# slothfulxtx/Texture-GS

Hardware: AMD Instinct MI355X
Metric: fwd+bwd views/sec @800x800, 300k Gaussians + 1024^2 texture; HBM GB/s vs roofline (higher is better)
Workload: dtype f32; 1 GPU; c3: N=300000 Gaussians, cubemap 6x1024x1024x3 f32, 800x800, fwd+bwd, sh_degree 3; parallelism=views sharded dp1, view_pipeline=3 HIP streams, order=accumulate, forwards begun one view per stream ahead, grad_allreduce=none (1 GPU)

## Files before the change

### texture-gs_amd/build.py

```python
import os
import subprocess
import sys

HERE = os.path.dirname(os.path.abspath(__file__))
ROOT = os.path.dirname(HERE)
CSRC = os.path.join(HERE, "csrc")
OBJ = os.path.join(HERE, "build")
LIB = os.path.join(HERE, os.environ.get("TEXGS_LIB_NAME", "libtexgs.so"))
OBJ = os.path.join(HERE, os.environ.get("TEXGS_OBJ_DIR", "build"))
HIPCC = os.environ.get("HIPCC", "/opt/rocm/bin/hipcc")

COMMON = ["--offload-arch=gfx950", "-O3", "-std=c++17", "-fPIC", "-I" + os.path.join(ROOT, "include"),
          "-I" + CSRC, "-Wall"]
UNITS = {
    "preprocess.hip": ["-ffp-contract=off"],
    "binning.hip": [],
    "render.hip": ["-munsafe-fp-atomics", "-ffp-contract=fast", "-fno-slp-vectorize"],
    "loss.hip": [],
    "selftest.hip": [],
    "uvnet.hip": [],
    "uvmap.hip": ["-munsafe-fp-atomics"],
    "points.hip": ["-ffp-contract=off"],
    "cubetex.hip": ["-munsafe-fp-atomics"],
    "density.hip": ["-ffp-contract=off"],
    "metrics.hip": ["-ffp-contract=off"],
    "optim.hip": ["-ffp-contract=off"],
    "mlp.hip": [],
    "present.hip": ["-ffp-contract=off"],
    "abi.hip": [],
}
HEADERS = [os.path.join(CSRC, "common.h"), os.path.join(CSRC, "wave_ops.h"), os.path.join(CSRC, "render_bwd_body.h"),
           os.path.join(ROOT, "include", "texgs.h"), os.path.join(ROOT, "include", "texgs_optim.h"),
           os.path.join(ROOT, "include", "texgs_multiview.h"), os.path.join(ROOT, "include", "texgs_mlp.h"),
           os.path.join(ROOT, "include", "texgs_present.h")]


def build_id():
    import hashlib
    h = hashlib.sha256()
    files = sorted(os.path.join(CSRC, f) for f in os.listdir(CSRC) if f.endswith((".hip", ".h"))) \
        + [os.path.join(ROOT, "include", f) for f in ("texgs.h", "texgs_optim.h", "texgs_multiview.h", "texgs_mlp.h", "texgs_present.h")]
    for f in files:
        h.update(os.path.basename(f).encode())
        h.update(open(f, "rb").read())
    h.update(repr((COMMON[:4], sorted(UNITS.items()), os.environ.get("TEXGS_EXTRA_FLAGS", ""))).encode())
    return h.hexdigest()[:16]


def _newer(src_list, target):
    if not os.path.exists(target):
        return True
    t = os.path.getmtime(target)
    return any(os.path.getmtime(s) > t for s in src_list)


def build(force=False, verbose=False):
    os.makedirs(OBJ, exist_ok=True)
    objs = []
    bid = build_id()
    idfile = os.path.join(OBJ, "build_id.txt")
    stale_id = not os.path.exists(idfile) or open(idfile).read().strip() != bid
    for src, flags in UNITS.items():
        sp = os.path.join(CSRC, src)
        op = os.path.join(OBJ, src.replace(".hip", ".o"))
        objs.append(op)
        if src == "abi.hip":
            flags = flags + ['-DTEXGS_BUILD_ID="%s"' % bid]
        if force or _newer([sp] + HEADERS + [os.path.abspath(__file__)], op) or (src == "abi.hip" and stale_id):
            cmd = [HIPCC] + COMMON + flags + os.environ.get("TEXGS_EXTRA_FLAGS", "").split() + ["-c", sp, "-o", op]
            if verbose:
                print(" ".join(cmd), flush=True)
            subprocess.check_call(cmd)
    if force or _newer(objs, LIB):
        cmd = [HIPCC, "--offload-arch=gfx950", "-shared", "-fPIC", "-o", LIB] + objs
        if verbose:
            print(" ".join(cmd), flush=True)
        subprocess.check_call(cmd)
    with open(idfile, "w") as f:
        f.write(bid + "\n")
    return LIB


if __name__ == "__main__":
    print(build(force="--force" in sys.argv, verbose="--verbose" in sys.argv or True))
```

### texture-gs_amd/csrc/abi.hip

```cpp
#include "common.h"
#include <stdio.h>
#include <stdlib.h>

#include <mutex>
#include <vector>

namespace {

thread_local char g_err[512] = "";

struct EvRec { int kid; hipEvent_t a, b; };
std::mutex g_prof_mu;
bool g_prof_on = false;
uint32_t g_prof_mask = 0xFFFFFFFFu;
std::vector<EvRec> g_prof_log;
std::vector<hipEvent_t> g_prof_free;

hipEvent_t prof_event() {
    if (!g_prof_free.empty()) { hipEvent_t e = g_prof_free.back(); g_prof_free.pop_back(); return e; }
    hipEvent_t e = nullptr;
    return hipEventCreate(&e) == hipSuccess ? e : nullptr;
}

struct ProfScope {
    int kid; hipStream_t s; hipEvent_t a; bool on;
    ProfScope(int k, hipStream_t st) : kid(k), s(st), a(nullptr), on(false) {
        std::lock_guard<std::mutex> l(g_prof_mu);
        if (g_prof_on && ((g_prof_mask >> k) & 1u)) { a = prof_event(); on = a != nullptr; if (on) (void)hipEventRecord(a, s); }
    }
    ~ProfScope() {
        if (!on) return;
        std::lock_guard<std::mutex> l(g_prof_mu);
        hipEvent_t b = prof_event();
        if (!b) { g_prof_free.push_back(a); return; }
        (void)hipEventRecord(b, s);
        g_prof_log.push_back({kid, a, b});
    }
};

int fail(const char* where, hipError_t e) {
    snprintf(g_err, sizeof(g_err), "%s: %s", where, hipGetErrorString(e));
    return (int)e ? (int)e : -1;
}

int fail_msg(const char* msg) {
    snprintf(g_err, sizeof(g_err), "%s", msg);
    return -1;
}

int launched(const char* where, hipError_t st, hipStream_t s, bool debug) {
    if (st == hipSuccess && debug) st = hipStreamSynchronize(s);
    return st == hipSuccess ? 0 : fail(where, st);
}

int validate_frame(const TexGSFrame* f) {
    if (!f) return fail_msg("frame is NULL");
    if (f->image_height <= 0 || f->image_width <= 0) return fail_msg("image size must be positive");
    if (f->image_width > 65535 * TEXGS_TILE || f->image_height > 65535 * TEXGS_TILE) return fail_msg("image too large");
    {
        const long long tx = (f->image_width + TEXGS_TILE - 1) / TEXGS_TILE, ty = (f->image_height + TEXGS_TILE - 1) / TEXGS_TILE;
        if (tx * ty > (1ll << 24)) return fail_msg("image too large: more than 2^24 tiles");
    }
    if (f->sh_degree < 0 || f->sh_degree > 3) return fail_msg("sh_degree must be in [0,3]");
    if (f->num_gaussians < 0) return fail_msg("num_gaussians < 0");
    if (f->tex_res <= 0) return fail_msg("tex_res must be positive");
    if (f->tex_res > 7168) return fail_msg("tex_res > 7168: the blend kernels address texels with 32-bit byte offsets (6 R^2 x 12 B < 2^32)");
    if (!f->bg || !f->viewmatrix || !f->projmatrix || !f->campos) return fail_msg("frame device pointers must be non-NULL");
    return 0;
}

}

extern "C" {

int texgs_abi_version(void) { return TEXGS_ABI_VERSION; }

#ifndef TEXGS_BUILD_ID
#define TEXGS_BUILD_ID "unknown"
#endif
const char* texgs_build_id(void) { return TEXGS_BUILD_ID; }

const char* texgs_last_error(void) { return g_err; }

size_t texgs_scan_temp_bytes(int32_t num_gaussians) { return scan_temp_bytes(num_gaussians); }

size_t texgs_sort_temp_bytes(uint32_t num_rendered, uint32_t num_tiles) { return sort_temp_bytes(num_rendered, num_tiles); }

size_t texgs_tex_bin_count(int32_t tex_res) { return tex_bin_count(tex_res); }

int texgs_preprocess_forward(const TexGSFrame* frame, const TexGSInputs* in, TexGSGeom* geom, void* stream) {
    if (int r = validate_frame(frame)) return r;
    if (!in || !geom) return fail_msg("NULL argument");
    if (frame->num_gaussians == 0) return 0;
    if (!in->means3D || !in->opacities) return fail_msg("per-Gaussian input pointer is NULL");
    if (in->texture && (!in->uvs || !in->gradient_uvs)) return fail_msg("uvs / gradient_uvs are required with a texture");
    if (in->cov3D_precomp && in->texture) return fail_msg("cov3D_precomp is an input of the untextured surface only (texture must be NULL)");
    if (!in->cov3D_precomp && (!in->scales || !in->rotations)) return fail_msg("scales and rotations (or cov3D_precomp) are required");
    if (geom->scan_temp_bytes < scan_temp_bytes(frame->num_gaussians)) return fail_msg("scan_temp too small");
    hipStream_t s = (hipStream_t)stream;
    const CamConst c = make_cam(frame);
    hipError_t st;
    { ProfScope p(TEXGS_K_PREPROCESS_FWD, s); st = launch_preprocess_fwd(c, frame, in, geom, s); }
    return launched("preprocess_fwd", st, s, frame->debug);
}

static int depth_sort_scan(const TexGSGeom* geom, int32_t num_gaussians, hipStream_t s, bool debug) {
    if (num_gaussians == 0) return 0;
    hipError_t st;
    { ProfScope p(TEXGS_K_SCAN, s); st = launch_depth_sort_scan(geom, num_gaussians, s); }
    return launched("depth sort / scan", st, s, debug);
}

size_t texgs_num_rendered_words(int32_t num_gaussians) {
    return num_gaussians <= 0 ? 0 : 3 * (((size_t)num_gaussians + TG_BLOCK - 1) / TG_BLOCK);
}
int texgs_num_rendered_begin(const TexGSGeom* geom, int32_t num_gaussians, uint32_t* host_pinned, size_t host_words, int32_t sort_first,
                             void* stream) {
    if (!geom || !host_pinned) return fail_msg("NULL argument");
    if (num_gaussians <= 0) return 0;
// ... 32 lines not shown
    const CamConst c = make_cam(frame);
    if (img->tex_bin_count && in->texture && !counters_zeroed) {
        hipError_t e = hipMemsetAsync(img->tex_bin_count, 0, sizeof(uint32_t) * 2 * tex_bin_count(c.R), s);
        if (e != hipSuccess) return fail("tex_bin_count memset", e);
    }
    hipError_t st;
    { ProfScope p(TEXGS_K_RENDER_FWD, s); st = launch_render_fwd(c, frame, in, geom, bin, img, s); }
    return launched("render_fwd", st, s, frame->debug);
}

int texgs_render_forward(const TexGSFrame* frame, const TexGSInputs* in, const TexGSGeom* geom,
                         const TexGSBinning* bin, TexGSImage* img, void* stream) {
    return render_forward_impl(frame, in, geom, bin, img, stream, false);
}

int texgs_bin_sort_render_forward(const TexGSFrame* frame, const TexGSInputs* in, const TexGSGeom* geom,
                                  TexGSBinning* bin, TexGSImage* img, void* stream) {
    if (int r = validate_frame(frame)) return r;
    if (!in || !geom || !bin || !img) return fail_msg("NULL argument");
    hipStream_t s = (hipStream_t)stream;
    const CamConst c = make_cam(frame);
    hipError_t st;
    if (bin->num_rendered > 0) {
        if (bin->sort_temp_bytes < sort_temp_bytes(bin->num_rendered, (uint32_t)(c.tiles_x * c.tiles_y))) return fail_msg("sort_temp too small");
        { ProfScope p(TEXGS_K_DUPLICATE, s); st = launch_duplicate(c, geom, bin, s); }
        if (int r = launched("duplicate_with_keys", st, s, frame->debug)) return r;
        { ProfScope p(TEXGS_K_SORT, s); st = launch_sort(c, geom, bin, s); }
        if (int r = launched("tile sort", st, s, frame->debug)) return r;
    }
    { ProfScope p(TEXGS_K_RANGES, s);
      st = launch_ranges(c, bin, img->tex_bin_count, img->tex_bin_count ? 2 * (int)tex_bin_count(c.R) : 0, s); }
    if (int r = launched("tile_ranges", st, s, frame->debug)) return r;
    return render_forward_impl(frame, in, geom, bin, img, stream, true);
}

int texgs_backward_render(const TexGSFrame* frame, const TexGSInputs* in, const TexGSGeom* geom,
                          const TexGSBinning* bin, const TexGSImage* img, TexGSGrads* grads, void* stream) {
    if (int r = validate_frame(frame)) return r;
    if (!in || !geom || !bin || !img || !grads) return fail_msg("NULL argument");
    if (!(grads->want & TEXGS_WANT_ALL)) return fail_msg("TexGSGrads.want is empty: ask for TEXGS_WANT_TEXTURE and / or TEXGS_WANT_GAUSSIANS");
    if ((grads->want & TEXGS_WANT_GAUSSIANS) && !grads->acc) return fail_msg("acc must be allocated (zero-filled) when Gaussian gradients are wanted");
    if ((grads->want & TEXGS_WANT_TEXTURE) && in->texture && !grads->dL_dtexture) return fail_msg("dL_dtexture must be allocated (zero-filled) when the texture gradient is wanted");
    if (!img->survivors || !img->surv_qmask || !img->surv_count)
        return fail_msg("the forward of this call left no survivor lists (TexGSImage.survivors / surv_qmask / surv_count were NULL): "
                        "run the forward with them to be able to run its backward");
    hipStream_t s = (hipStream_t)stream;
    const CamConst c = make_cam(frame);
    if (bin->num_rendered > 0) {
        hipError_t st;
        { ProfScope p(TEXGS_K_RENDER_BWD, s); st = launch_render_bwd(c, frame, in, geom, bin, img, grads, s); }
        if (int r = launched("render_bwd", st, s, frame->debug)) return r;
        if (tex_bins_enabled(c, in, img, grads)) {
            { ProfScope p(TEXGS_K_TEXGRAD_REDUCE, s); st = launch_texgrad_reduce(c, img, grads, s); }
            return launched("texgrad_reduce", st, s, frame->debug);
        }
    }
    return 0;
}

int texgs_backward_preprocess(const TexGSFrame* frame, const TexGSInputs* in, const TexGSGeom* geom, TexGSGrads* grads,
                              void* stream) {
    if (int r = validate_frame(frame)) return r;
    if (!in || !geom || !grads) return fail_msg("NULL argument");
    if (!(grads->want & TEXGS_WANT_GAUSSIANS)) return 0;
    if (!grads->acc) return fail_msg("acc must be allocated");
    if (in->cov3D_precomp && !grads->dL_dcov3D) return fail_msg("dL_dcov3D is required with cov3D_precomp");
    if (grads->dL_dvd_residue && (grads->accumulate & (TEXGS_ACC_SHS | TEXGS_ACC_MEANS3D)) != (TEXGS_ACC_SHS | TEXGS_ACC_MEANS3D))
        return fail_msg("dL_dvd_residue needs TEXGS_ACC_SHS and TEXGS_ACC_MEANS3D in accumulate: texgs_sh_flush adds into both");
    hipStream_t s = (hipStream_t)stream;
    const CamConst c = make_cam(frame);
    hipError_t st;
    { ProfScope p(TEXGS_K_PREPROCESS_BWD, s); st = launch_preprocess_bwd(c, frame, in, geom, grads, s); }
    return launched("preprocess_bwd", st, s, frame->debug);
}

int texgs_backward(const TexGSFrame* frame, const TexGSInputs* in, const TexGSGeom* geom,
                   const TexGSBinning* bin, const TexGSImage* img, TexGSGrads* grads, void* stream) {
    if (int r = texgs_backward_render(frame, in, geom, bin, img, grads, stream)) return r;
    return texgs_backward_preprocess(frame, in, geom, grads, stream);
}

int texgs_profile_enable(int on) {
    std::lock_guard<std::mutex> l(g_prof_mu);
    g_prof_on = on != 0;
    if (!g_prof_on) {
        for (auto& r : g_prof_log) { g_prof_free.push_back(r.a); g_prof_free.push_back(r.b); }
        g_prof_log.clear();
    }
    return 0;
}

int texgs_profile_select(uint32_t kernel_mask) {
    std::lock_guard<std::mutex> l(g_prof_mu);
    g_prof_mask = kernel_mask;
    return 0;
}

int texgs_profile_read(float* ms_sum_host, uint32_t* launches_host) {
    if (!ms_sum_host || !launches_host) return fail_msg("NULL argument");
    std::lock_guard<std::mutex> l(g_prof_mu);
    for (auto& r : g_prof_log) {
        hipError_t e = hipEventSynchronize(r.b);
        if (e != hipSuccess) return fail("profile event sync", e);
        float ms = 0.f;
        e = hipEventElapsedTime(&ms, r.a, r.b);
        if (e != hipSuccess) return fail("profile elapsed", e);
        if (r.kid >= 0 && r.kid < TEXGS_NUM_KERNELS) { ms_sum_host[r.kid] += ms; launches_host[r.kid] += 1; }
        g_prof_free.push_back(r.a); g_prof_free.push_back(r.b);
    }
    g_prof_log.clear();
    return 0;
}

int texgs_rgb_alpha_loss(const float* image, const float* gt_image, const float* alpha, const float* gt_alpha,
                         int32_t H, int32_t W, float lambda_dssim, float lambda_alpha, float* scratch, float* sums,
                         float* dL_dimage, float* dL_dalpha, void* stream) {
    if (!image || !gt_image || !scratch || !sums || !dL_dimage) return fail_msg("NULL argument");
    if (H <= 0 || W <= 0) return fail_msg("image size must be positive");
    hipStream_t s = (hipStream_t)stream;
    return launched("rgb_alpha_loss", launch_rgb_alpha_loss(image, gt_image, alpha, gt_alpha, H, W, lambda_dssim, lambda_alpha, scratch,
                                                            sums, dL_dimage, dL_dalpha, s), s, false);
}

int texgs_geom_losses(const float* norm, const float* gt_norm, const float* gt_image, const float* mask, const float* depth,
                      const float* gt_depth, int32_t H, int32_t W, float lambda_norm, float lambda_smooth, float gamma,
                      float lambda_depth, float* sums, float* dL_dnorm, float* dL_ddepth, void* stream) {
    if (!sums) return fail_msg("NULL argument");
    if (H <= 0 || W <= 0 || !(gamma > 0.f)) return fail_msg("image size and gamma must be positive");
    if (lambda_norm != 0.f && (!norm || !gt_norm || !dL_dnorm)) return fail_msg("norm term needs norm, gt_norm, dL_dnorm");
    if (lambda_smooth != 0.f && (!norm || !gt_image || !dL_dnorm)) return fail_msg("smoothness term needs norm, gt_image, dL_dnorm");
    if (lambda_depth != 0.f && (!depth || !gt_depth || !dL_ddepth)) return fail_msg("depth term needs depth, gt_depth, dL_ddepth");
    hipStream_t s = (hipStream_t)stream;
    return launched("geom_losses", launch_geom_losses(norm, gt_norm, gt_image, mask, depth, gt_depth, H, W, lambda_norm, lambda_smooth,
                                                      gamma, lambda_depth, sums, dL_dnorm, dL_ddepth, s), s, false);
}

int texgs_norm_from_depth(const float* depth, const float* viewmatrix, float tanfovx, float tanfovy, int32_t H, int32_t W,
                          float threshold, float* out_norm, float* out_mask, void* stream) {
    if (!depth || !viewmatrix || !out_norm || !out_mask) return fail_msg("NULL argument");
    if (H <= 0 || W <= 0) return fail_msg("image size must be positive");
    hipStream_t s = (hipStream_t)stream;
    return launched("norm_from_depth", launch_norm_from_depth(depth, viewmatrix, tanfovx, tanfovy, H, W, threshold, out_norm, out_mask, s),
                    s, false);
}

static int check_uvnet(const TexGSUVNet* net, int32_t precision) {
    if (precision != TEXGS_UV_FP32 && precision != TEXGS_UV_BF16X3 && precision != TEXGS_UV_MIXED)
        return fail_msg("precision must be TEXGS_UV_FP32, TEXGS_UV_BF16X3 or TEXGS_UV_MIXED");
    if (net->hidden != 128) return fail_msg("the UV-map kernels support the shipped UVNet shape only (hidden width 128)");
    if (!net->W1 || !net->W2 || !net->W3 || !net->W4 || !net->W5 || !net->emb) return fail_msg("weight pointer is NULL");
    return 0;
}

size_t texgs_uv_packed_bytes(int32_t precision) { return uv_packed_bytes(precision); }

int texgs_uv_pack(const TexGSUVNet* net, int32_t precision, void* packed, void* stream) {
    if (!net || !packed) return fail_msg("NULL argument");
    if (int r = check_uvnet(net, precision)) return r;
    hipStream_t s = (hipStream_t)stream;
    return launched("uv_pack", launch_uv_pack(net, precision, packed, s), s, false);
}

int texgs_uv_taylor_packed(const TexGSUVNet* net, int32_t precision, const void* packed, const float* xyz, int32_t N, float* uvs,
                           float* grad_uvs, void* stream) {
    if (!net || !packed) return fail_msg("NULL argument");
    if (int r = check_uvnet(net, precision)) return r;
    if (N < 0) return fail_msg("N < 0");
    if (N > 0 && (!xyz || !uvs || !grad_uvs)) return fail_msg("NULL argument");
    hipStream_t s = (hipStream_t)stream;
    return launched("uv_taylor", launch_uv_taylor_packed(net, precision, packed, xyz, N, uvs, grad_uvs, s), s, false);
}

size_t texgs_uv_backward_temp_bytes(int32_t N) { return uv_backward_temp_bytes(N < 0 ? 0 : N); }

int texgs_uv_backward(const TexGSUVNet* net, int32_t precision, const float* xyz, const float* g_uvs, int32_t N, const TexGSUVNetGrad* out,
                      void* temp, void* stream) {
    if (!net || !out || !temp) return fail_msg("NULL argument");
    if (int r = check_uvnet(net, precision)) return r;
    if (N < 0) return fail_msg("N < 0");
    if (N > 0 && (!xyz || !g_uvs)) return fail_msg("NULL argument");
    hipStream_t s = (hipStream_t)stream;
    return launched("uv_backward", launch_uv_backward(net, xyz, g_uvs, N, out, temp, precision != TEXGS_UV_FP32, s), s, false);
}

static int check_hashgrid(const TexGSHashGrid* g, uint32_t* n_params) {
    if (!g) return fail_msg("grid is NULL");
    float sc[TEXGS_HASHGRID_MAX_LEVELS];
    uint32_t r[TEXGS_HASHGRID_MAX_LEVELS], sz[TEXGS_HASHGRID_MAX_LEVELS], off[TEXGS_HASHGRID_MAX_LEVELS];
    switch (hashgrid_levels(g, sc, r, sz, off, n_params)) {
    case 0: return 0;
    case -1: return fail_msg("hash grid: n_levels must be in [1, 16]");
    case -2: return fail_msg("hash grid: n_features must be 4");
    case -3: return fail_msg("hash grid: log2_hashmap_size must be in [1, 24]");
    case -4: return fail_msg("hash grid: base_resolution must be >= 1 and per_level_scale in [1, 16]");
// ... 341 lines not shown
```

### texture-gs_amd/csrc/preprocess.hip

```cpp
#include "common.h"

namespace {

struct Frame {
    float V[16];
    float P[16];
    float cam[3];
};

__device__ __forceinline__ Frame load_frame(const float* vm, const float* pm, const float* cp) {
    Frame f;
#pragma unroll
    for (int i = 0; i < 16; ++i) { f.V[i] = vm[i]; f.P[i] = pm[i]; }
    f.cam[0] = cp[0]; f.cam[1] = cp[1]; f.cam[2] = cp[2];
    return f;
}

struct Geo {
    bool  valid;
    float m[3], t[3];
    float hx, hy, hw, pw, xy[2];
    float q[4], s[3], R[9], M[9], S[6];
    float txc, tyc; bool clx, cly;
    float J00, J02, J11, J12, T0[3], T1[3];
// ... 548 lines not shown
                dBm[k * 2 + cc] = g.K[0 * 3 + k] * dG[0 * 2 + cc] + g.K[1 * 3 + k] * dG[1 * 2 + cc] + g.K[2 * 3 + k] * dG[2 * 2 + cc];
        float dtz = dBm[0] / C.fx + dBm[3] / C.fy;
        float dgt[2];
#pragma unroll
        for (int cc = 0; cc < 2; ++cc)
            dgt[cc] = A[R_G2 + cc] - (dBm[0 * 2 + cc] * tx + dBm[1 * 2 + cc] * ty + dBm[2 * 2 + cc] * tz);
#pragma unroll
        for (int k = 0; k < 3; ++k) dt[k] -= dBm[k * 2 + 0] * g.gx + dBm[k * 2 + 1] * g.gy;
        const float dax = dgt[0] / C.fx, day = dgt[1] / C.fy;
        const float dot_a_nv = dax * g.nv[0] + day * g.nv[1];
        dtz += dot_a_nv / g.sdot;
        float dnv[3] = {tz * dax / g.sdot, tz * day / g.sdot, 0.f};
        const float ds = -tz * dot_a_nv / (g.sdot * g.sdot);
        dnv[0] += ds * tx; dnv[1] += ds * ty; dnv[2] += ds * tz;
        dt[0] += ds * g.nv[0]; dt[1] += ds * g.nv[1]; dt[2] += ds * g.nv[2] + dtz;
#pragma unroll
        for (int k = 0; k < 3; ++k)
            dn[k] += dnv[0] * WR(F, 0, k) + dnv[1] * WR(F, 1, k) + dnv[2] * WR(F, 2, k);
    }
#pragma unroll
    for (int k = 0; k < 3; ++k) {
        const float on = (g.kmin == k) ? g.sign : 0.0f;
        dR[0 + k] += on * dn[0]; dR[3 + k] += on * dn[1]; dR[6 + k] += on * dn[2];
    }

    if constexpr (DEFER) {
        d_vd_res[3 * i + 0] = (na > 0) ? A[R_VD] : 0.f; d_vd_res[3 * i + 1] = (na > 0) ? A[R_VD + 1] : 0.f;
        d_vd_res[3 * i + 2] = (na > 0) ? A[R_VD + 2] : 0.f;
    } else if (d_shs && na > 0) {
        float b[15], bx[15], by[15], bz[15];
#pragma unroll
        for (int k = 0; k < 15; ++k) { b[k] = 0.f; bx[k] = 0.f; by[k] = 0.f; bz[k] = 0.f; }
        sh_basis(C.sh_degree, g.dir[0], g.dir[1], g.dir[2], b);
        sh_basis_grad(C.sh_degree, g.dir[0], g.dir[1], g.dir[2], bx, by, bz);
        float* sp = s_sh + threadIdx.x * row;
        const float v0 = A[R_VD], v1 = A[R_VD + 1], v2 = A[R_VD + 2];
        float ddx = 0.f, ddy = 0.f, ddz = 0.f;
#pragma unroll
        for (int k = 0; k < 15; ++k) {
            if (k < na) {
                const float w = sp[3 * k + 0] * v0 + sp[3 * k + 1] * v1 + sp[3 * k + 2] * v2;
                ddx += bx[k] * w; ddy += by[k] * w; ddz += bz[k] * w;
                sp[3 * k + 0] = b[k] * v0; sp[3 * k + 1] = b[k] * v1; sp[3 * k + 2] = b[k] * v2;
            }
        }
        for (int k = 3 * na; k < row; ++k) sp[k] = 0.f;
        const float dd = g.dir[0] * ddx + g.dir[1] * ddy + g.dir[2] * ddz;
        dm[0] += (ddx - g.dir[0] * dd) / g.dlen;
        dm[1] += (ddy - g.dir[1] * dd) / g.dlen;
        dm[2] += (ddz - g.dir[2] * dd) / g.dlen;
    }

#pragma unroll
    for (int k = 0; k < 3; ++k) dm[k] += dt[0] * F.V[k * 4 + 0] + dt[1] * F.V[k * 4 + 1] + dt[2] * F.V[k * 4 + 2];
    OUT(TEXGS_ACC_MEANS3D, d_means[3 * i + 0], dm[0]); OUT(TEXGS_ACC_MEANS3D, d_means[3 * i + 1], dm[1]); OUT(TEXGS_ACC_MEANS3D, d_means[3 * i + 2], dm[2]);
    if constexpr (COV) {
        OUT(TEXGS_ACC_COV3D, d_cov6[6 * i + 0], dS[0]); OUT(TEXGS_ACC_COV3D, d_cov6[6 * i + 1], dS[1] + dS[3]);
        OUT(TEXGS_ACC_COV3D, d_cov6[6 * i + 2], dS[2] + dS[6]); OUT(TEXGS_ACC_COV3D, d_cov6[6 * i + 3], dS[4]);
        OUT(TEXGS_ACC_COV3D, d_cov6[6 * i + 4], dS[5] + dS[7]); OUT(TEXGS_ACC_COV3D, d_cov6[6 * i + 5], dS[8]);
    }
    if constexpr (!COV) { OUT(TEXGS_ACC_SCALES, d_scales[3 * i + 0], dscale[0]); OUT(TEXGS_ACC_SCALES, d_scales[3 * i + 1], dscale[1]); OUT(TEXGS_ACC_SCALES, d_scales[3 * i + 2], dscale[2]); }

    if constexpr (!COV) {
    const float r = g.q[0], x = g.q[1], y = g.q[2], z = g.q[3];
    OUT(TEXGS_ACC_ROTATIONS, d_rots[4 * i + 0], 2.0f * (-z * dR[1] + y * dR[2] + z * dR[3] - x * dR[5] - y * dR[6] + x * dR[7]));
    OUT(TEXGS_ACC_ROTATIONS, d_rots[4 * i + 1], 2.0f * (y * dR[1] + z * dR[2] + y * dR[3] - 2.0f * x * dR[4] - r * dR[5] + z * dR[6] + r * dR[7] - 2.0f * x * dR[8]));
    OUT(TEXGS_ACC_ROTATIONS, d_rots[4 * i + 2], 2.0f * (-2.0f * y * dR[0] + x * dR[1] + r * dR[2] + x * dR[3] + z * dR[5] - r * dR[6] + z * dR[7] - 2.0f * y * dR[8]));
    OUT(TEXGS_ACC_ROTATIONS, d_rots[4 * i + 3], 2.0f * (-2.0f * z * dR[0] - r * dR[1] + x * dR[2] + r * dR[3] - 2.0f * z * dR[4] + y * dR[5] + x * dR[6] + y * dR[7]));
    }
#undef OUT
    }
    if constexpr (!DEFER) if (d_shs) {
        if (na == 0 || (live && !visible)) {
            if (live) for (int k = 0; k < row; ++k) s_sh[threadIdx.x * row + k] = 0.f;
        }
        __syncthreads();
        if (accumulate & TEXGS_ACC_SHS) sh_rows_out<BLOCK, true>(d_shs + first, s_sh, count, vec);
        else sh_rows_out<BLOCK, false>(d_shs + first, s_sh, count, vec);
    }
}

constexpr int FL_BLOCK = 256;
constexpr int FL_MAX = TEXGS_SH_FLUSH_MAX_VIEWS;

struct ShFlushArgs {
    TexGSShFlushView v[FL_MAX];
    int32_t count;
};

__global__ void __launch_bounds__(FL_BLOCK)
k_sh_flush(ShFlushArgs a, int N, int K, const float* __restrict__ means, const float* __restrict__ shs,
           float* __restrict__ d_shs, float* __restrict__ d_means) {
    extern __shared__ __attribute__((aligned(16))) float s_row[];
    const int i = blockIdx.x * FL_BLOCK + threadIdx.x;
    const bool live = i < N;
    const int row = 3 * K;
    const size_t first = (size_t)blockIdx.x * FL_BLOCK * row;
    const int count = (int)min((size_t)FL_BLOCK * row, (size_t)N * row - first);
    const bool vec = (((size_t)d_shs) & 15) == 0;
    for (int k = threadIdx.x; k < count; k += FL_BLOCK) s_row[k] = shs[first + k];
    __syncthreads();
    float sp[45];
#pragma unroll
    for (int k = 0; k < 45; ++k) sp[k] = (live && k < row) ? s_row[threadIdx.x * row + k] : 0.f;
    __syncthreads();
    for (int k = threadIdx.x; k < count; k += FL_BLOCK) s_row[k] = d_shs[first + k];
    __syncthreads();
    if (live) {
        const float m[3] = {means[3 * i + 0], means[3 * i + 1], means[3 * i + 2]};
        float* gp = s_row + threadIdx.x * row;
        float dm[3] = {d_means[3 * i + 0], d_means[3 * i + 1], d_means[3 * i + 2]};
        bool any = false;
        for (int v = 0; v < a.count; ++v) {
            const float* __restrict__ res = a.v[v].residue;
            const float v0 = res[3 * i + 0], v1 = res[3 * i + 1], v2 = res[3 * i + 2];
            const int deg = a.v[v].sh_degree;
            const int na = deg > 0 ? sh_active(deg, K) : 0;
            if ((v0 == 0.f && v1 == 0.f && v2 == 0.f) || na == 0) continue;
            const float* __restrict__ cp = a.v[v].campos;
            const float cam[3] = {cp[0], cp[1], cp[2]};
            float raw[3], dir[3];
            const float dlen = view_direction(m, cam, raw, dir);
            float b[15], bx[15], by[15], bz[15];
#pragma unroll
            for (int k = 0; k < 15; ++k) { b[k] = 0.f; bx[k] = 0.f; by[k] = 0.f; bz[k] = 0.f; }
            sh_basis(deg, dir[0], dir[1], dir[2], b);
            sh_basis_grad(deg, dir[0], dir[1], dir[2], bx, by, bz);
            float ddx = 0.f, ddy = 0.f, ddz = 0.f;
#pragma unroll
            for (int k = 0; k < 15; ++k) {
                if (k < na) {
                    const float w = sp[3 * k + 0] * v0 + sp[3 * k + 1] * v1 + sp[3 * k + 2] * v2;
                    ddx += bx[k] * w; ddy += by[k] * w; ddz += bz[k] * w;
                    gp[3 * k + 0] = gp[3 * k + 0] + b[k] * v0; gp[3 * k + 1] = gp[3 * k + 1] + b[k] * v1;
                    gp[3 * k + 2] = gp[3 * k + 2] + b[k] * v2;
                }
            }
            const float dd = dir[0] * ddx + dir[1] * ddy + dir[2] * ddz;
            dm[0] += (ddx - dir[0] * dd) / dlen;
            dm[1] += (ddy - dir[1] * dd) / dlen;
            dm[2] += (ddz - dir[2] * dd) / dlen;
            any = true;
        }
        if (any) { d_means[3 * i + 0] = dm[0]; d_means[3 * i + 1] = dm[1]; d_means[3 * i + 2] = dm[2]; }
    }
    __syncthreads();
    sh_rows_out<FL_BLOCK, false>(d_shs + first, s_row, count, vec);
}

__global__ void __launch_bounds__(TG_BLOCK)
k_mark_visible(int N, const float* __restrict__ vm, const float* __restrict__ means, uint8_t* __restrict__ visible) {
    const int i = blockIdx.x * TG_BLOCK + threadIdx.x;
    if (i >= N) return;
    const float tz = vm[2] * means[3 * i] + vm[6] * means[3 * i + 1] + vm[10] * means[3 * i + 2] + vm[14];
    visible[i] = tz > TG_NEAR_Z ? 1 : 0;
}

}

hipError_t launch_preprocess_fwd(const CamConst& c, const TexGSFrame* f, const TexGSInputs* in, TexGSGeom* g, hipStream_t s) {
    if (c.N <= 0) return hipSuccess;
    const int blocks = (c.N + TG_BLOCK - 1) / TG_BLOCK;
    const size_t lds = (in->shs && c.sh_degree > 0) ? (size_t)TG_BLOCK * 3 * c.sh_coeffs * sizeof(float) : 0;
    int hdr_words = 0;
    uint32_t* hdr = bin_header_ptr(g, c.N, &hdr_words);
#define K1_LAUNCH(COV) hipLaunchKernelGGL(k_preprocess_fwd<COV>, dim3(blocks), dim3(TG_BLOCK), lds, s, c, f->viewmatrix, f->projmatrix, f->campos, \
                       in->means3D, in->shs, in->opacities, in->scales, in->rotations, in->uvs, in->gradient_uvs, in->color_offset, \
                       in->cov3D_precomp, reinterpret_cast<float4*>(g->rec_test), reinterpret_cast<float4*>(g->rec_shade), g->depth, g->radii, \
                       reinterpret_cast<uint2*>(g->rect), g->tiles_touched, bin_block_sums_ptr(g, c.N), hdr, hdr_words)
    if (in->cov3D_precomp) K1_LAUNCH(true); else K1_LAUNCH(false);
#undef K1_LAUNCH
    return hipGetLastError();
}

hipError_t launch_preprocess_bwd(const CamConst& c, const TexGSFrame* f, const TexGSInputs* in, const TexGSGeom* g,
                           TexGSGrads* gr, hipStream_t s) {
    if (c.N <= 0) return hipSuccess;
#define K8_LAUNCH(COV, DEFER, BLOCK, LDS) hipLaunchKernelGGL((k_preprocess_bwd<COV, DEFER, BLOCK>), dim3((c.N + BLOCK - 1) / BLOCK), dim3(BLOCK), LDS, s, \
                       c, f->viewmatrix, f->projmatrix, f->campos, \
                       in->means3D, in->shs, in->opacities, in->scales, in->rotations, in->gradient_uvs, in->cov3D_precomp, \
                       g->radii, gr->acc, gr->dL_dmeans3D, gr->dL_dmeans2D, gr->dL_dshs, gr->dL_dopacities, gr->dL_dscales, \
                       gr->dL_drotations, gr->dL_duvs, gr->dL_dcolor_offset, gr->dL_dcov3D, gr->dL_dvd_residue, gr->accumulate)
    if (gr->dL_dvd_residue) {
        if (in->cov3D_precomp) K8_LAUNCH(true, true, K8_DEFER_BLOCK, 0); else K8_LAUNCH(false, true, K8_DEFER_BLOCK, 0);
    } else {
        const size_t lds = gr->dL_dshs ? (size_t)K8_BLOCK * 3 * c.sh_coeffs * sizeof(float) : 0;
        if (in->cov3D_precomp) K8_LAUNCH(true, false, K8_BLOCK, lds); else K8_LAUNCH(false, false, K8_BLOCK, lds);
    }
#undef K8_LAUNCH
    return hipGetLastError();
}

hipError_t launch_sh_flush(int N, int K, const float* means3D, const float* shs, float* dL_dshs, float* dL_dmeans3D,
                           const TexGSShFlushView* views, int count, hipStream_t s) {
    if (count < 0 || count > FL_MAX) return hipErrorInvalidValue;
    if (N <= 0 || count == 0) return hipSuccess;
    ShFlushArgs a;
    for (int k = 0; k < FL_MAX; ++k) a.v[k] = k < count ? views[k] : TexGSShFlushView{nullptr, nullptr, 0, 0};
// ... 13 lines not shown
```

### texture-gs_amd/texgs/_lib.py

```python
import contextlib
import ctypes as C
import os

_HERE = os.path.dirname(os.path.abspath(__file__))
LIB_PATH = os.environ.get("TEXGS_LIB") or os.path.join(os.path.dirname(_HERE), "libtexgs.so")

ABI_VERSION = 19
TILE = 16
REC_TEST_FLOATS = 8
REC_SHADE_FLOATS = 20
TEXBIN_RECORD_FLOATS = 4
RESV_WORDS = 192
ACC_FLOATS = 32
WANT_TEXTURE, WANT_GAUSSIANS, WANT_ALL = 1, 2, 3

_fp = C.c_void_p


class Frame(C.Structure):
    _fields_ = [("image_height", C.c_int32), ("image_width", C.c_int32), ("tanfovx", C.c_float),
                ("tanfovy", C.c_float), ("scale_modifier", C.c_float), ("sh_degree", C.c_int32),
                ("sh_coeffs", C.c_int32), ("tex_res", C.c_int32), ("num_gaussians", C.c_int32),
                ("debug", C.c_int32), ("bg", _fp), ("viewmatrix", _fp), ("projmatrix", _fp), ("campos", _fp)]


class Inputs(C.Structure):
    _fields_ = [("means3D", _fp), ("shs", _fp), ("opacities", _fp), ("scales", _fp), ("rotations", _fp),
                ("uvs", _fp), ("gradient_uvs", _fp), ("texture", _fp), ("color_offset", _fp), ("cov3D_precomp", _fp)]


class Geom(C.Structure):
    _fields_ = [("rec_test", _fp), ("rec_shade", _fp), ("depth", _fp), ("radii", _fp), ("rect", _fp), ("tiles_touched", _fp),
                ("offsets", _fp), ("scan_temp", _fp), ("scan_temp_bytes", C.c_size_t)]


class Binning(C.Structure):
    _fields_ = [("num_rendered", C.c_uint32), ("keys_unsorted", _fp), ("keys_sorted", _fp), ("point_list", _fp),
                ("ranges", _fp), ("tile_order", _fp), ("sort_temp", _fp), ("sort_temp_bytes", C.c_size_t)]


class Image(C.Structure):
    _fields_ = [("out_color", _fp), ("out_depth", _fp), ("out_norm", _fp), ("out_alpha", _fp),
                ("final_T", _fp), ("n_contrib", _fp), ("tex_bin_count", _fp),
                ("survivors", _fp), ("surv_qmask", _fp), ("surv_count", _fp), ("tex_bin_resv", _fp)]


class Grads(C.Structure):
    _fields_ = [("dL_dcolor", _fp), ("dL_ddepth", _fp), ("dL_dnorm", _fp), ("dL_dalpha", _fp), ("acc", _fp),
                ("dL_dmeans3D", _fp), ("dL_dmeans2D", _fp), ("dL_dshs", _fp), ("dL_dopacities", _fp),
                ("dL_dscales", _fp), ("dL_drotations", _fp), ("dL_duvs", _fp), ("dL_dtexture", _fp),
                ("dL_dcolor_offset", _fp), ("dL_dcov3D", _fp), ("want", C.c_uint32), ("tex_bins", _fp), ("tex_bin_cursor", _fp), ("tex_bin_base", _fp),
                ("tex_rec_cap", C.c_uint32),
                ("accumulate", C.c_int32), ("dL_dvd_residue", _fp)]


class UVNetStruct(C.Structure):
    _fields_ = [(n, _fp) for n in ("W1", "b1", "W2", "b2", "emb", "W3", "b3", "W4", "b4", "W5", "b5", "xyz_offset", "xyz_scale")] \
        + [("hidden", C.c_int32)]


class HashGridStruct(C.Structure):
    _fields_ = [("n_levels", C.c_int32), ("n_features", C.c_int32), ("log2_hashmap_size", C.c_int32), ("base_resolution", C.c_float),
                ("per_level_scale", C.c_float)]


HASHGRID_MAX_LEVELS = 16
HASHGRID_FEATURES = 4


class UVNetGradStruct(C.Structure):
    _fields_ = [(n, _fp) for n in ("dW1", "db1", "dW2", "db2", "dW3", "db3", "dW4", "db4", "dW5", "db5")]


DENSITY_KEEP, DENSITY_CLONE, DENSITY_CLONE_KEPT, DENSITY_SPLIT, DENSITY_CHILD = 1, 2, 4, 8, 16
DENSITY_ROW = {"copy": 0, "moment": 1, "scaling": 2, "xyz": 3}
DENSITY_MAX_ROWS = 24
METRICS_ROW = 16


class DensityPlanStruct(C.Structure):
    _fields_ = [("accum", _fp), ("denom", _fp), ("scaling", _fp), ("opacity", _fp), ("n", C.c_int32), ("max_grad", C.c_float),
                ("min_opacity", C.c_float), ("dense_scale", C.c_float), ("big_scale", C.c_float), ("densify", C.c_int32),
                ("use_big", C.c_int32)]


class DensityRowStruct(C.Structure):
    _fields_ = [("src", _fp), ("dst", _fp), ("width", C.c_int32), ("kind", C.c_int32)]


class DensityMoveStruct(C.Structure):
    _fields_ = [("row", DensityRowStruct * DENSITY_MAX_ROWS), ("rows", C.c_int32), ("n", C.c_int32), ("action", _fp), ("rank", _fp),
                ("n_kept", C.c_int32), ("n_clone", C.c_int32), ("n_split", C.c_int32), ("n_child", C.c_int32), ("scaling", _fp),
                ("rotation", _fp), ("noise", _fp)]


UV_PRECISION = {"fp32": 0, "bf16x3": 1, "mixed": 2}


_P = C.POINTER
_i32, _u32, _f32, _size, _vp = C.c_int32, C.c_uint32, C.c_float, C.c_size_t, C.c_void_p
_frame5 = [_P(Frame), _P(Inputs), _P(Geom), _P(Binning), _P(Image)]
SIGNATURES = {
    "texgs_abi_version": (C.c_int, []),
    "texgs_build_id": (C.c_char_p, []),
    "texgs_last_error": (C.c_char_p, []),
    "texgs_scan_temp_bytes": (_size, [_i32]),
    "texgs_sort_temp_bytes": (_size, [_u32, _u32]),
    "texgs_tex_bin_count": (_size, [_i32]),
    "texgs_preprocess_forward": (C.c_int, [_P(Frame), _P(Inputs), _P(Geom), _vp]),
    "texgs_num_rendered_words": (_size, [_i32]),
    "texgs_num_rendered_begin": (C.c_int, [_P(Geom), _i32, _vp, _size, _i32, _vp]),
    "texgs_num_rendered_reduce": (C.c_int, [_vp, _i32, _P(_u32), _P(C.c_uint64)]),
    "texgs_depth_sort_scan": (C.c_int, [_P(Geom), _i32, _vp]),
    "texgs_bin_sort_render_forward": (C.c_int, _frame5 + [_vp]),
    "texgs_render_forward": (C.c_int, _frame5 + [_vp]),
    "texgs_backward": (C.c_int, _frame5 + [_P(Grads), _vp]),
    "texgs_backward_render": (C.c_int, _frame5 + [_P(Grads), _vp]),
    "texgs_backward_preprocess": (C.c_int, [_P(Frame), _P(Inputs), _P(Geom), _P(Grads), _vp]),
    "texgs_profile_enable": (C.c_int, [C.c_int]),
    "texgs_profile_select": (C.c_int, [_u32]),
    "texgs_profile_read": (C.c_int, [_P(_f32), _P(_u32)]),
    "texgs_rgb_alpha_loss": (C.c_int, [_vp] * 4 + [_i32, _i32, _f32, _f32] + [_vp] * 5),
    "texgs_geom_losses": (C.c_int, [_vp] * 6 + [_i32, _i32, _f32, _f32, _f32, _f32] + [_vp] * 4),
    "texgs_norm_from_depth": (C.c_int, [_vp, _vp, _f32, _f32, _i32, _i32, _f32, _vp, _vp, _vp]),
    "texgs_uv_packed_bytes": (_size, [_i32]),
    "texgs_uv_pack": (C.c_int, [_P(UVNetStruct), _i32, _vp, _vp]),
    "texgs_uv_taylor_packed": (C.c_int, [_P(UVNetStruct), _i32, _vp, _vp, _i32, _vp, _vp, _vp]),
    "texgs_uv_backward_temp_bytes": (_size, [_i32]),
    "texgs_uv_backward": (C.c_int, [_P(UVNetStruct), _i32, _vp, _vp, _i32, _P(UVNetGradStruct), _vp, _vp]),
    "texgs_hashgrid_levels": (C.c_int, [_P(HashGridStruct), _vp, _vp, _vp, _vp, _P(_u32)]),
    "texgs_hashgrid_forward": (C.c_int, [_P(HashGridStruct), _vp, _vp, _i32, _vp, _vp]),
    "texgs_hashgrid_backward_temp_bytes": (_size, [_P(HashGridStruct), _i32]),
    "texgs_hashgrid_backward": (C.c_int, [_P(HashGridStruct), _vp, _vp, _vp, _i32, _vp, _vp, _vp, _vp]),
    "texgs_chamfer_nn_temp_bytes": (_size, [_i32]),
    "texgs_chamfer_nn": (C.c_int, [_vp, _i32, _vp, _i32, _vp, _vp, _vp, _vp]),
    "texgs_knn3_temp_bytes": (_size, [_i32]),
    "texgs_knn3_mean_dist2": (C.c_int, [_vp, _i32, _vp, _vp, _vp]),
    "texgs_fps_temp_bytes": (_size, [_i32, _i32]),
    "texgs_farthest_points": (C.c_int, [_vp, _i32, _i32, _i32, _vp, _vp, _vp]),
    "texgs_cube_sample": (C.c_int, [_vp, _i32, _i32, _vp, _i32, _i32, _i32, _vp, _vp]),
    "texgs_cube_latlong": (C.c_int, [_vp, _i32, _i32, _i32, _i32, _i32, _vp, _vp]),
    "texgs_cube_sample_backward": (C.c_int, [_vp, _i32, _i32, _vp, _i32, _vp, _vp, _vp, _vp]),
    "texgs_cube_sample_nearest_backward": (C.c_int, [_i32, _i32, _vp, _i32, _vp, _vp, _vp]),
    "texgs_density_stats": (C.c_int, [_vp, _vp, _i32, _vp, _vp, _vp, _vp]),
    "texgs_density_plan_temp_bytes": (_size, [_i32]),
    "texgs_density_plan": (C.c_int, [_P(DensityPlanStruct), _vp, _vp, _vp, _vp, _vp]),
    "texgs_density_move": (C.c_int, [_P(DensityMoveStruct), _vp]),
    "texgs_eval_metrics_temp_bytes": (_size, [_i32, _i32]),
    "texgs_eval_metrics": (C.c_int, [_vp] * 5 + [_i32, _i32, _i32, _vp, _vp, _vp]),
    "texgs_selftest_waveops": (C.c_int, [_vp, _vp, _vp]),
    "texgs_mark_visible": (C.c_int, [_P(Frame), _vp, _vp, _vp]),
}
EXPORTS = list(SIGNATURES)
KERNEL_NAMES = ["preprocess_fwd", "scan", "duplicate", "sort", "ranges", "render_fwd", "render_bwd", "preprocess_bwd",
                "texgrad_reduce"]

_lib = None


def load():
    global _lib
    if _lib is not None:
        return _lib
    if not os.path.exists(LIB_PATH):
        raise RuntimeError(
            f"libtexgs.so not found at {LIB_PATH}: build it with `python texture-gs_amd/build.py` "
            "(hipcc --offload-arch=gfx950). There is no CPU fallback for the rasterizer.")
    lib = C.CDLL(LIB_PATH)
    missing = [n for n in EXPORTS if not hasattr(lib, n)]
    if missing:
        raise RuntimeError(f"libtexgs.so at {LIB_PATH} does not export {', '.join(missing)}; rebuild it with "
                           "`python texture-gs_amd/build.py`")
    for name, (restype, argtypes) in SIGNATURES.items():
        fn = getattr(lib, name)
        fn.restype, fn.argtypes = restype, argtypes
    v = lib.texgs_abi_version()
    if v != ABI_VERSION:
        raise RuntimeError(f"libtexgs.so ABI version {v} != expected {ABI_VERSION}; rebuild it")
    global BUILD_ID
    BUILD_ID = lib.texgs_build_id().decode()
    if not os.environ.get("TEXGS_LIB"):
        want = tree_build_id()
        if want is not None and BUILD_ID != want:
            raise RuntimeError(f"libtexgs.so was built from other sources (build id {BUILD_ID}, this tree is {want}); "
                               "rebuild it with `python texture-gs_amd/build.py`")
    _lib = lib
    return lib


BUILD_ID = None


def tree_build_id():
    import importlib.util
    path = os.path.join(os.path.dirname(_HERE), "build.py")
    if not os.path.exists(path):
        return None
    spec = importlib.util.spec_from_file_location("texgs_build_script", path)
    mod = importlib.util.module_from_spec(spec)
    spec.loader.exec_module(mod)
    return mod.build_id()


def check(rc, what):
    if rc != 0:
        msg = load().texgs_last_error().decode("utf-8", "replace")
        raise RuntimeError(f"{what} failed (code {rc}): {msg}")


def call(fn, *args):
    rc = fn(*args)
    if rc != 0:
        check(rc, fn.__name__)


def ptr(t):
    return None if t is None else t.data_ptr()


@contextlib.contextmanager
def on(device):
    import torch
    with torch.cuda.device(device):
        yield torch.cuda.current_stream(device).cuda_stream


def profile_enable(on: bool, only=None):
    mask = 0xFFFFFFFF if only is None else sum(1 << KERNEL_NAMES.index(n) for n in only)
    call(load().texgs_profile_select, mask)
    call(load().texgs_profile_enable, 1 if on else 0)


def profile_read():
    n = len(KERNEL_NAMES)
    ms = (C.c_float * n)()
    cnt = (C.c_uint32 * n)()
    call(load().texgs_profile_read, ms, cnt)
    return {KERNEL_NAMES[i]: (float(ms[i]), int(cnt[i])) for i in range(n)}
```

Before: 1048 views/s.

## Bound profiler events in a fixed ring and vectorise SH flush loads

Replaces the unbounded per-launch event log with a fixed ring of preallocated event pairs that is harvested as it fills and counts dropped brackets. Separately, the SH flush kernel now stages SH rows and their gradients into shared memory with float4 loads, keeping six loads in flight per thread. It also preloads the per-view residues and the means into registers before the view loop. The profiler part only runs when profiling is on. The flush part adds register pressure from the residue array and the in-flight vectors.

Result: no change. 1047 views/s (-0.0%).

```diff
diff --git a/include/texgs_profile.h b/include/texgs_profile.h
--- /dev/null
+++ b/include/texgs_profile.h
@@ -0,0 +1,20 @@
+#ifndef TEXGS_PROFILE_H
+#define TEXGS_PROFILE_H
+
+#include "texgs.h"
+
+#ifdef __cplusplus
+extern "C" {
+#endif
+
+#define TEXGS_PROFILE_RING_PAIRS 32
+
+int texgs_profile_dropped(uint32_t* dropped_host);
+
+int texgs_profile_live_events(void);
+
+#ifdef __cplusplus
+}
+#endif
+
+#endif
diff --git a/texture-gs_amd/build.py b/texture-gs_amd/build.py
--- a/texture-gs_amd/build.py
+++ b/texture-gs_amd/build.py
@@ -30,16 +30,18 @@
     "abi.hip": [],
 }
 HEADERS = [os.path.join(CSRC, "common.h"), os.path.join(CSRC, "wave_ops.h"), os.path.join(CSRC, "render_bwd_body.h"),
+           os.path.join(CSRC, "prof_ring.h"),
            os.path.join(ROOT, "include", "texgs.h"), os.path.join(ROOT, "include", "texgs_optim.h"),
            os.path.join(ROOT, "include", "texgs_multiview.h"), os.path.join(ROOT, "include", "texgs_mlp.h"),
-           os.path.join(ROOT, "include", "texgs_present.h")]
+           os.path.join(ROOT, "include", "texgs_present.h"), os.path.join(ROOT, "include", "texgs_profile.h")]
 
 
 def build_id():
     import hashlib
     h = hashlib.sha256()
     files = sorted(os.path.join(CSRC, f) for f in os.listdir(CSRC) if f.endswith((".hip", ".h"))) \
-        + [os.path.join(ROOT, "include", f) for f in ("texgs.h", "texgs_optim.h", "texgs_multiview.h", "texgs_mlp.h", "texgs_present.h")]
+        + [os.path.join(ROOT, "include", f) for f in ("texgs.h", "texgs_optim.h", "texgs_multiview.h", "texgs_mlp.h", "texgs_present.h",
+                                                            "texgs_profile.h")]
     for f in files:
         h.update(os.path.basename(f).encode())
         h.update(open(f, "rb").read())
diff --git a/texture-gs_amd/csrc/abi.hip b/texture-gs_amd/csrc/abi.hip
--- a/texture-gs_amd/csrc/abi.hip
+++ b/texture-gs_amd/csrc/abi.hip
@@ -1,40 +1,43 @@
 #include "common.h"
+#include "prof_ring.h"
+#include "texgs_profile.h"
 #include <stdio.h>
 #include <stdlib.h>
 
 #include <mutex>
-#include <vector>
 
 namespace {
 
 thread_local char g_err[512] = "";
 
-struct EvRec { int kid; hipEvent_t a, b; };
+struct HipEventApi {
+    using Event = hipEvent_t;
+    bool create(Event* e) { *e = nullptr; return hipEventCreate(e) == hipSuccess; }
+    void destroy(Event e) { (void)hipEventDestroy(e); }
+    bool record(Event e, hipStream_t s) { return hipEventRecord(e, s) == hipSuccess; }
+    bool done(Event e) { return hipEventQuery(e) == hipSuccess; }
+    bool wait(Event e) { last = hipEventSynchronize(e); return last == hipSuccess; }
+    bool elapsed(float* ms, Event a, Event b) { last = hipEventElapsedTime(ms, a, b); return last == hipSuccess; }
+    hipError_t last = hipSuccess;
+};
 std::mutex g_prof_mu;
 bool g_prof_on = false;
 uint32_t g_prof_mask = 0xFFFFFFFFu;
-std::vector<EvRec> g_prof_log;
-std::vector<hipEvent_t> g_prof_free;
-
-hipEvent_t prof_event() {
-    if (!g_prof_free.empty()) { hipEvent_t e = g_prof_free.back(); g_prof_free.pop_back(); return e; }
-    hipEvent_t e = nullptr;
-    return hipEventCreate(&e) == hipSuccess ? e : nullptr;
-}
+static_assert(PROF_RING_PAIRS == TEXGS_PROFILE_RING_PAIRS, "texgs_profile.h states the ring's size too");
+HipEventApi g_prof_api;
+ProfRing<HipEventApi, PROF_RING_PAIRS, TEXGS_NUM_KERNELS> g_prof_ring;
+int g_prof_dev = -1;
 
 struct ProfScope {
-    int kid; hipStream_t s; hipEvent_t a; bool on;
-    ProfScope(int k, hipStream_t st) : kid(k), s(st), a(nullptr), on(false) {
+    hipStream_t s; int slot; uint32_t gen;
+    ProfScope(int k, hipStream_t st) : s(st), slot(-1), gen(0) {
         std::lock_guard<std::mutex> l(g_prof_mu);
-        if (g_prof_on && ((g_prof_mask >> k) & 1u)) { a = prof_event(); on = a != nullptr; if (on) (void)hipEventRecord(a, s); }
+        if (g_prof_on && ((g_prof_mask >> k) & 1u)) { gen = g_prof_ring.gen; slot = g_prof_ring.open(g_prof_api, k, s); }
     }
     ~ProfScope() {
-        if (!on) return;
+        if (slot < 0) return;
         std::lock_guard<std::mutex> l(g_prof_mu);
-        hipEvent_t b = prof_event();
-        if (!b) { g_prof_free.push_back(a); return; }
-        (void)hipEventRecord(b, s);
-        g_prof_log.push_back({kid, a, b});
+        g_prof_ring.close(g_prof_api, slot, gen, s);
     }
 };
 
@@ -233,11 +236,17 @@
 
 int texgs_profile_enable(int on) {
     std::lock_guard<std::mutex> l(g_prof_mu);
+    if (on) {
+        int dev = -1;
+        hipError_t e = hipGetDevice(&dev);
+        if (e != hipSuccess) return fail("profile enable", e);
+        if (g_prof_ring.created && dev != g_prof_dev) g_prof_ring.destroy(g_prof_api);
+        if (!g_prof_ring.create(g_prof_api)) return fail_msg("profile enable: the runtime could not create the bracket's events");
+        g_prof_dev = dev;
+    } else {
+        g_prof_ring.reset();
+    }
     g_prof_on = on != 0;
-    if (!g_prof_on) {
-        for (auto& r : g_prof_log) { g_prof_free.push_back(r.a); g_prof_free.push_back(r.b); }
-        g_prof_log.clear();
-    }
     return 0;
 }
 
@@ -250,17 +259,20 @@
 int texgs_profile_read(float* ms_sum_host, uint32_t* launches_host) {
     if (!ms_sum_host || !launches_host) return fail_msg("NULL argument");
     std::lock_guard<std::mutex> l(g_prof_mu);
-    for (auto& r : g_prof_log) {
-        hipError_t e = hipEventSynchronize(r.b);
-        if (e != hipSuccess) return fail("profile event sync", e);
-        float ms = 0.f;
-        e = hipEventElapsedTime(&ms, r.a, r.b);
-        if (e != hipSuccess) return fail("profile elapsed", e);
-        if (r.kid >= 0 && r.kid < TEXGS_NUM_KERNELS) { ms_sum_host[r.kid] += ms; launches_host[r.kid] += 1; }
-        g_prof_free.push_back(r.a); g_prof_free.push_back(r.b);
-    }
-    g_prof_log.clear();
-    return 0;
+    if (!g_prof_ring.read(g_prof_api, ms_sum_host, launches_host)) return fail("profile event read", g_prof_api.last);
+    return 0;
+}
+
+int texgs_profile_dropped(uint32_t* dropped_host) {
+    if (!dropped_host) return fail_msg("NULL argument");
+    std::lock_guard<std::mutex> l(g_prof_mu);
+    g_prof_ring.read_dropped(dropped_host);
+    return 0;
+}
+
+int texgs_profile_live_events(void) {
+    std::lock_guard<std::mutex> l(g_prof_mu);
+    return g_prof_ring.live_events();
 }
 
 int texgs_rgb_alpha_loss(const float* image, const float* gt_image, const float* alpha, const float* gt_alpha,
diff --git a/texture-gs_amd/csrc/preprocess.hip b/texture-gs_amd/csrc/preprocess.hip
--- a/texture-gs_amd/csrc/preprocess.hip
+++ b/texture-gs_amd/csrc/preprocess.hip
@@ -654,6 +654,33 @@
 
 constexpr int FL_BLOCK = 256;
 constexpr int FL_MAX = TEXGS_SH_FLUSH_MAX_VIEWS;
+constexpr int FL_INFLIGHT = 6;
+
+template <int BLOCK>
+__device__ __forceinline__ void sh_rows_in(float* s, const float* __restrict__ g, int count, bool vec) {
+    constexpr int U = FL_INFLIGHT;
+    static_assert(U == 6, "the statement below names six vectors");
+    const int tid = (int)threadIdx.x;
+    int done = 0;
+    if (vec) {
+        const int n4 = count >> 2;
+        const float4* __restrict__ g4 = reinterpret_cast<const float4*>(g);
+        float4* s4 = reinterpret_cast<float4*>(s);
+        for (int k = tid; k < n4; k += U * BLOCK) {
+            float4 v[U];
+#pragma unroll
+            for (int u = 0; u < U; ++u) v[u] = g4[min(k + u * BLOCK, n4 - 1)];
+            asm volatile("" :: "v"(v[0].x), "v"(v[0].y), "v"(v[0].z), "v"(v[0].w), "v"(v[1].x), "v"(v[1].y), "v"(v[1].z), "v"(v[1].w),
+                         "v"(v[2].x), "v"(v[2].y), "v"(v[2].z), "v"(v[2].w), "v"(v[3].x), "v"(v[3].y), "v"(v[3].z), "v"(v[3].w),
+                         "v"(v[4].x), "v"(v[4].y), "v"(v[4].z), "v"(v[4].w), "v"(v[5].x), "v"(v[5].y), "v"(v[5].z), "v"(v[5].w)
+                         : "memory");
+#pragma unroll
+            for (int u = 0; u < U; ++u) s4[min(k + u * BLOCK, n4 - 1)] = v[u];
+        }
+        done = n4 << 2;
+    }
+    for (int k = done + tid; k < count; k += BLOCK) s[k] = g[k];
+}
 
 struct ShFlushArgs {
     TexGSShFlushView v[FL_MAX];
@@ -670,22 +697,35 @@
     const size_t first = (size_t)blockIdx.x * FL_BLOCK * row;
     const int count = (int)min((size_t)FL_BLOCK * row, (size_t)N * row - first);
     const bool vec = (((size_t)d_shs) & 15) == 0;
-    for (int k = threadIdx.x; k < count; k += FL_BLOCK) s_row[k] = shs[first + k];
+    float rv[FL_MAX][3];
+#pragma unroll
+    for (int v = 0; v < FL_MAX; ++v) {
+        const bool on = live && v < a.count;
+        const float* __restrict__ res = a.v[v].residue;
+#pragma unroll
+        for (int c = 0; c < 3; ++c) rv[v][c] = on ? res[3 * (size_t)i + c] : 0.f;
+    }
+    float m[3], dm[3];
+#pragma unroll
+    for (int c = 0; c < 3; ++c) { m[c] = live ? means[3 * (size_t)i + c] : 0.f; dm[c] = live ? d_means[3 * (size_t)i + c] : 0.f; }
+    sh_rows_in<FL_BLOCK>(s_row, shs + first, count, (((size_t)shs) & 15) == 0);
     __syncthreads();
     float sp[45];
 #pragma unroll
     for (int k = 0; k < 45; ++k) sp[k] = (live && k < row) ? s_row[threadIdx.x * row + k] : 0.f;
     __syncthreads();
-    for (int k = threadIdx.x; k < count; k += FL_BLOCK) s_row[k] = d_shs[first + k];
+    sh_rows_in<FL_BLOCK>(s_row, d_shs + first, count, vec);
     __syncthreads();
     if (live) {
-        const float m[3] = {means[3 * i + 0], means[3 * i + 1], means[3 * i + 2]};
         float* gp = s_row + threadIdx.x * row;
-        float dm[3] = {d_means[3 * i + 0], d_means[3 * i + 1], d_means[3 * i + 2]};
         bool any = false;
+#pragma unroll 1
         for (int v = 0; v < a.count; ++v) {
-            const float* __restrict__ res = a.v[v].residue;
-            const float v0 = res[3 * i + 0], v1 = res[3 * i + 1], v2 = res[3 * i + 2];
+            const float v0 = rv[0][0], v1 = rv[0][1], v2 = rv[0][2];
+#pragma unroll
+            for (int u = 0; u + 1 < FL_MAX; ++u) {
+                rv[u][0] = rv[u + 1][0]; rv[u][1] = rv[u + 1][1]; rv[u][2] = rv[u + 1][2];
+            }
             const int deg = a.v[v].sh_degree;
             const int na = deg > 0 ? sh_active(deg, K) : 0;
             if ((v0 == 0.f && v1 == 0.f && v2 == 0.f) || na == 0) continue;
diff --git a/texture-gs_amd/csrc/prof_ring.h b/texture-gs_amd/csrc/prof_ring.h
--- /dev/null
+++ b/texture-gs_amd/csrc/prof_ring.h
@@ -0,0 +1,110 @@
+#pragma once
+#include <stdint.h>
+
+constexpr int PROF_RING_PAIRS = 32;
+
+template <class Api, int PAIRS, int KERNELS>
+struct ProfRing {
+    using Event = typename Api::Event;
+    enum State : uint8_t { FREE = 0, OPEN = 1, CLOSED = 2, DEAD = 3 };
+    struct Slot { Event a, b; int kid; State st; };
+
+    Slot slot[PAIRS];
+    bool created = false;
+    int head = 0;
+    int used = 0;
+    uint32_t gen = 0;
+    float ms_sum[KERNELS] = {};
+    uint32_t launches[KERNELS] = {};
+    uint32_t dropped[KERNELS] = {};
+
+    bool create(Api& api) {
+        if (created) return true;
+        for (int k = 0; k < PAIRS; ++k) {
+            slot[k].st = FREE; slot[k].kid = -1;
+            const bool okA = api.create(&slot[k].a);
+            const bool okB = okA && api.create(&slot[k].b);
+            if (!okB) {
+                if (okA) api.destroy(slot[k].a);
+                for (int j = 0; j < k; ++j) { api.destroy(slot[j].a); api.destroy(slot[j].b); }
+                return false;
+            }
+        }
+        head = used = 0;
+        created = true;
+        return true;
+    }
+
+    void destroy(Api& api) {
+        if (!created) return;
+        for (int k = 0; k < PAIRS; ++k) { api.destroy(slot[k].a); api.destroy(slot[k].b); }
+        created = false; head = used = 0; ++gen;
+    }
+
+    void reset() {
+        for (int k = 0; k < PAIRS; ++k) { slot[k].st = FREE; slot[k].kid = -1; }
+        head = used = 0; ++gen;
+        for (int k = 0; k < KERNELS; ++k) { ms_sum[k] = 0.f; launches[k] = 0; dropped[k] = 0; }
+    }
+
+    void harvest(Api& api) {
+        while (used > 0) {
+            Slot& s = slot[head];
+            if (s.st == OPEN || (s.st == CLOSED && !api.done(s.b))) return;
+            take(api, s);
+        }
+    }
+
+    template <class Stream>
+    int open(Api& api, int kid, Stream stream) {
+        if (!created) { if (kid >= 0 && kid < KERNELS) ++dropped[kid]; return -1; }
+        if (used == PAIRS) harvest(api);
+        if (used == PAIRS) { if (kid >= 0 && kid < KERNELS) ++dropped[kid]; return -1; }
+        const int k = (head + used) % PAIRS;
+        if (!api.record(slot[k].a, stream)) { if (kid >= 0 && kid < KERNELS) ++dropped[kid]; return -1; }
+        ++used;
+        slot[k].kid = kid; slot[k].st = OPEN;
+        return k;
+    }
+
+    template <class Stream>
+    void close(Api& api, int k, uint32_t g, Stream stream) {
+        if (k < 0 || g != gen || slot[k].st != OPEN) return;
+        if (api.record(slot[k].b, stream)) { slot[k].st = CLOSED; return; }
+        if (slot[k].kid >= 0 && slot[k].kid < KERNELS) ++dropped[slot[k].kid];
+        slot[k].st = DEAD;
+    }
+
+    int live_events() const {
+        int n = 0;
+        for (int j = 0; j < used; ++j) n += slot[(head + j) % PAIRS].st == CLOSED ? 2 : 1;
+        return n;
+    }
+
+    bool read(Api& api, float* ms_out, uint32_t* launches_out) {
+        bool ok = true;
+        while (ok && used > 0 && slot[head].st != OPEN) {
+            Slot& s = slot[head];
+            ok = (s.st == DEAD || api.wait(s.b)) && take(api, s);
+        }
+        for (int k = 0; k < KERNELS; ++k) {
+            ms_out[k] += ms_sum[k]; launches_out[k] += launches[k];
+            ms_sum[k] = 0.f; launches[k] = 0;
+        }
+        return ok;
+    }
+
+    void read_dropped(uint32_t* dropped_out) {
+        for (int k = 0; k < KERNELS; ++k) { dropped_out[k] += dropped[k]; dropped[k] = 0; }
+    }
+
+private:
+    bool take(Api& api, Slot& s) {
+        float ms = 0.f;
+        const bool ok = s.st == DEAD || api.elapsed(&ms, s.a, s.b);
+        if (ok && s.st == CLOSED && s.kid >= 0 && s.kid < KERNELS) { ms_sum[s.kid] += ms; launches[s.kid] += 1; }
+        s.st = FREE; s.kid = -1;
+        head = (head + 1) % PAIRS; --used;
+        return ok;
+    }
+};
diff --git a/texture-gs_amd/texgs/_lib.py b/texture-gs_amd/texgs/_lib.py
--- a/texture-gs_amd/texgs/_lib.py
+++ b/texture-gs_amd/texgs/_lib.py
@@ -12,6 +12,7 @@
 TEXBIN_RECORD_FLOATS = 4
 RESV_WORDS = 192
 ACC_FLOATS = 32
+PROFILE_RING_PAIRS = 32
 WANT_TEXTURE, WANT_GAUSSIANS, WANT_ALL = 1, 2, 3
 
 _fp = C.c_void_p
@@ -152,6 +153,10 @@
     "texgs_mark_visible": (C.c_int, [_P(Frame), _vp, _vp, _vp]),
 }
 EXPORTS = list(SIGNATURES)
+PROFILE_SIGNATURES = {
+    "texgs_profile_dropped": (C.c_int, [_P(_u32)]),
+    "texgs_profile_live_events": (C.c_int, []),
+}
 KERNEL_NAMES = ["preprocess_fwd", "scan", "duplicate", "sort", "ranges", "render_fwd", "render_bwd", "preprocess_bwd",
                 "texgrad_reduce"]
 
@@ -167,11 +172,11 @@
             f"libtexgs.so not found at {LIB_PATH}: build it with `python texture-gs_amd/build.py` "
             "(hipcc --offload-arch=gfx950). There is no CPU fallback for the rasterizer.")
     lib = C.CDLL(LIB_PATH)
-    missing = [n for n in EXPORTS if not hasattr(lib, n)]
+    missing = [n for n in EXPORTS + list(PROFILE_SIGNATURES) if not hasattr(lib, n)]
     if missing:
         raise RuntimeError(f"libtexgs.so at {LIB_PATH} does not export {', '.join(missing)}; rebuild it with "
                            "`python texture-gs_amd/build.py`")
-    for name, (restype, argtypes) in SIGNATURES.items():
+    for name, (restype, argtypes) in list(SIGNATURES.items()) + list(PROFILE_SIGNATURES.items()):
         fn = getattr(lib, name)
         fn.restype, fn.argtypes = restype, argtypes
     v = lib.texgs_abi_version()
@@ -237,3 +242,13 @@
     cnt = (C.c_uint32 * n)()
     call(load().texgs_profile_read, ms, cnt)
     return {KERNEL_NAMES[i]: (float(ms[i]), int(cnt[i])) for i in range(n)}
+
+
+def profile_dropped():
+    cnt = (C.c_uint32 * len(KERNEL_NAMES))()
+    call(load().texgs_profile_dropped, cnt)
+    return {KERNEL_NAMES[i]: int(cnt[i]) for i in range(len(KERNEL_NAMES))}
+
+
+def profile_live_events():
+    return int(load().texgs_profile_live_events())
```
